# imironhead/ml_super_resolution

Hardware: AMD Instinct MI355X
Metric: VDSR-20 training patches/sec (41x41, batch 256 per GPU); fwd HR megapixels/sec alongside (higher is better)
Workload: dtype f32; 1 GPU; BASELINE configs[2]: VDSR 20-layer 3x3x64 residual, RGB, batch 256x41x41 per GPU, fwd+bwd+TF-Adam, random-init weights; global_batch=256, patch=41, parallelism=dp1

## Files before the change

ml_super_resolution_amd/csrc/conv_inst_c4.hip:

```cpp
#include "launchers.h"
namespace srx {
bool launch_conv_c4(const ConvKey& k, const ConvArgs& a, int grid, size_t lds, hipStream_t s, hipError_t* err) {
    SRX_CONV_CASE(3, 3, 4, 4, false, 2)
    SRX_CONV_CASE(3, 3, 4, 4, true, 2)
    SRX_CONV_CASE(3, 3, 4, 2, false, 2)
    SRX_CONV_CASE(3, 3, 4, 2, true, 2)
    SRX_CONV_CASE(3, 3, 4, 1, false, 2)
    SRX_CONV_CASE(5, 5, 4, 4, false, 2)
    SRX_CONV_CASE(5, 5, 4, 4, true, 2)
    SRX_CONV_CASE(5, 5, 4, 2, false, 2)
    SRX_CONV_CASE(5, 5, 4, 2, true, 2)
    SRX_CONV_CASE(9, 9, 4, 4, false, 2)
    SRX_CONV_CASE(9, 9, 4, 4, true, 2)
    return false;
}
}
```

ml_super_resolution_amd/csrc/conv_narrow.hip:

```cpp
#include "launchers.h"
namespace srx {
typedef float f32x3 __attribute__((ext_vector_type(3)));
typedef unsigned u32x3v __attribute__((ext_vector_type(3)));

template <int CTRL>
__device__ __forceinline__ float dpp_add(float v) {
    const int moved = __builtin_amdgcn_update_dpp(0, __float_as_int(v), CTRL, 0xf, 0xf, false);
    return v + __int_as_float(moved);
}

struct PixWalk {
    int n, oh, ow;
    __device__ __forceinline__ void init(unsigned p, int OH, int OW) {
        const unsigned t = p / (unsigned)OW;
        ow = (int)(p - t * (unsigned)OW);
        n = (int)(t / (unsigned)OH);
        oh = (int)(t - (unsigned)n * (unsigned)OH);
    }
    __device__ __forceinline__ void step16(int OH, int OW) { step(16, OH, OW); }
    __device__ __forceinline__ void step(int d, int OH, int OW) {
        ow += d;
        while (ow >= OW) {
            ow -= OW;
            oh += 1;
            if (oh == OH) { oh = 0; n += 1; }
        }
    }
};
template <int KH, int KW>
__device__ __forceinline__ void tap_offsets(int (&off)[KH * KW], const PixWalk& q, bool live, int H, int W, int pad_t, int pad_l,
                                            int PB, int lane_b) {
    const int centre = ((q.n * H + q.oh - pad_t) * W + (q.ow - pad_l)) * PB + lane_b;
    bool rok[KH], cok[KW];
#pragma unroll
    for (int kh = 0; kh < KH; ++kh) rok[kh] = live && (unsigned)(q.oh + kh - pad_t) < (unsigned)H;
#pragma unroll
    for (int kw = 0; kw < KW; ++kw) cok[kw] = (unsigned)(q.ow + kw - pad_l) < (unsigned)W;
#pragma unroll
    for (int kh = 0; kh < KH; ++kh)
#pragma unroll
        for (int kw = 0; kw < KW; ++kw)
            off[kh * KW + kw] = (rok[kh] && cok[kw]) ? centre + (kh * W + kw) * PB : kOobOffset;
}

template <int KH, int KW, int CIN, int CO>
__global__ __launch_bounds__(256) void conv_narrow_kernel(const ConvArgs a, long total_px, int iters) {
    static_assert(CIN == 64, "16 lanes x 4 channels per pixel");
    constexpr int TAPS = KH * KW;
    const int c4 = threadIdx.x & 15;
    const int sub = threadIdx.x >> 4;
    float wr[TAPS][4][CO];
#pragma unroll
    for (int t = 0; t < TAPS; ++t)
#pragma unroll
        for (int e = 0; e < 4; ++e)
#pragma unroll
            for (int c = 0; c < CO; ++c) wr[t][e][c] = a.w[((size_t)t * CIN + 4 * c4 + e) * CO + c];
    float bias[CO];
#pragma unroll
    for (int c = 0; c < CO; ++c) bias[c] = a.bias ? a.bias[c] : 0.0f;
    const __amdgpu_buffer_rsrc_t xrs = __builtin_amdgcn_make_buffer_rsrc(const_cast<float*>(a.x), 0,
                                                                         a.N * a.H * a.W * CIN * 4, 0x00020000);
    const unsigned p0 = blockIdx.x * (unsigned)iters * 16u + sub;
    PixWalk q;
    q.init(p0 < (unsigned)total_px ? p0 : 0u, a.OH, a.OW);
    for (int it = 0; it < iters; ++it, q.step16(a.OH, a.OW)) {
        const unsigned p = p0 + (unsigned)it * 16u;
        const bool live = p < (unsigned)total_px;
        int off[TAPS];
        tap_offsets<KH, KW>(off, q, live, a.H, a.W, a.pad_t, a.pad_l, CIN * 4, 16 * c4);
        f32x4 v[TAPS];
#pragma unroll
        for (int tp = 0; tp < TAPS; ++tp)
            v[tp] = __builtin_bit_cast(f32x4, __builtin_amdgcn_raw_buffer_load_b128(xrs, off[tp], 0, 0));
        float acc[CO];
#pragma unroll
        for (int c = 0; c < CO; ++c) acc[c] = 0.0f;
#pragma unroll
        for (int tp = 0; tp < TAPS; ++tp)
#pragma unroll
            for (int e = 0; e < 4; ++e)
#pragma unroll
                for (int c = 0; c < CO; ++c) acc[c] = fmaf(v[tp][e], wr[tp][e][c], acc[c]);
#pragma unroll
        for (int c = 0; c < CO; ++c) {
            float r = acc[c];
            r = dpp_add<0xB1>(r);
            r = dpp_add<0x4E>(r);
            r = dpp_add<0x124>(r);
            r = dpp_add<0x128>(r);
            acc[c] = r;
        }
        if (live && c4 < CO) {
            float r = (c4 == 0) ? acc[0] : (c4 == 1 ? acc[1 < CO ? 1 : 0] : acc[2 < CO ? 2 : 0]);
            r = act_apply(r + ((c4 == 0) ? bias[0] : (c4 == 1 ? bias[1 < CO ? 1 : 0] : bias[2 < CO ? 2 : 0])), a.act);
            const size_t o = (size_t)p * CO + c4;
            if (a.skip) r += a.skip[o];
            if (a.post_relu) r = act_apply(r, a.post_relu);
            a.y[o] = r;
        }
    }
}

template <int KH, int KW, bool NOUT, int CW = 64>
__global__ __launch_bounds__(256) void wgrad_narrow_kernel(const WgradArgs a, long total_px, int iters) {
    constexpr int TAPS = KH * KW, CN = 3;
    constexpr int LPP = CW / 4;
    constexpr int PPI = 256 / LPP;
    constexpr int NB = NOUT ? CN : 4;
    constexpr int NV = TAPS * 4 * CN + NB;
    __shared__ float red[4 * NV * LPP];
    const int c4 = threadIdx.x & (LPP - 1);
    const int sub = threadIdx.x / LPP;
    const int wave = threadIdx.x >> 6;
    float acc[NV];
#pragma unroll
    for (int i = 0; i < NV; ++i) acc[i] = 0.0f;
    const __amdgpu_buffer_rsrc_t xrs = __builtin_amdgcn_make_buffer_rsrc(
        const_cast<float*>(a.x), 0, a.N * a.H * a.W * (NOUT ? CW : CN) * 4, 0x00020000);
    const __amdgpu_buffer_rsrc_t drs = __builtin_amdgcn_make_buffer_rsrc(
        const_cast<float*>(a.dpre), 0, a.N * a.OH * a.OW * (NOUT ? CN : CW) * 4, 0x00020000);
    const unsigned p0 = blockIdx.x * (unsigned)iters * (unsigned)PPI + sub;
    PixWalk q;
    q.init(p0 < (unsigned)total_px ? p0 : 0u, a.OH, a.OW);
    for (int it = 0; it < iters; ++it, q.step(PPI, a.OH, a.OW)) {
        const unsigned p = p0 + (unsigned)it * (unsigned)PPI;
        const bool live = p < (unsigned)total_px;
        int off[TAPS];
        tap_offsets<KH, KW>(off, q, live, a.H, a.W, a.pad_t, a.pad_l, (NOUT ? CW : CN) * 4, NOUT ? 16 * c4 : 0);
        if constexpr (NOUT) {
            const f32x3 d = __builtin_bit_cast(f32x3, __builtin_amdgcn_raw_buffer_load_b96(drs, live ? (int)(p * CN * 4) : kOobOffset, 0, 0));
            f32x4 v[TAPS];
#pragma unroll
            for (int tp = 0; tp < TAPS; ++tp)
                v[tp] = __builtin_bit_cast(f32x4, __builtin_amdgcn_raw_buffer_load_b128(xrs, off[tp], 0, 0));
#pragma unroll
            for (int tp = 0; tp < TAPS; ++tp)
#pragma unroll
                for (int e = 0; e < 4; ++e)
#pragma unroll
                    for (int c = 0; c < CN; ++c) acc[(tp * 4 + e) * CN + c] = fmaf(v[tp][e], d[c], acc[(tp * 4 + e) * CN + c]);
#pragma unroll
            for (int c = 0; c < CN; ++c) acc[TAPS * 4 * CN + c] += d[c];
        } else {
            const f32x4 d = __builtin_bit_cast(f32x4, __builtin_amdgcn_raw_buffer_load_b128(
                drs, live ? (int)((p * CW + 4 * c4) * 4) : kOobOffset, 0, 0));
            f32x3 v[TAPS];
#pragma unroll
            for (int tp = 0; tp < TAPS; ++tp)
                v[tp] = __builtin_bit_cast(f32x3, __builtin_amdgcn_raw_buffer_load_b96(xrs, off[tp], 0, 0));
#pragma unroll
            for (int tp = 0; tp < TAPS; ++tp)
#pragma unroll
                for (int cn = 0; cn < CN; ++cn)
#pragma unroll
                    for (int e = 0; e < 4; ++e) acc[(tp * CN + cn) * 4 + e] = fmaf(v[tp][cn], d[e], acc[(tp * CN + cn) * 4 + e]);
#pragma unroll
            for (int e = 0; e < 4; ++e) acc[TAPS * 4 * CN + e] += d[e];
        }
    }
#pragma unroll
    for (int i = 0; i < NV; ++i) {
        float r = acc[i];
#pragma unroll
        for (int o = LPP; o < 64; o <<= 1) r += __shfl_xor(r, o);
        if (sub % (64 / LPP) == 0) red[(wave * NV + i) * LPP + c4] = r;
    }
    __syncthreads();
    float* part = a.part + (size_t)blockIdx.x * a.part_stride;
    const int wn = TAPS * CW * CN;
    for (int q = threadIdx.x; q < NV * LPP; q += 256) {
        const int i = q / LPP, l = q % LPP;
        const float r = (red[(0 * NV + i) * LPP + l] + red[(1 * NV + i) * LPP + l]) +
                        (red[(2 * NV + i) * LPP + l] + red[(3 * NV + i) * LPP + l]);
        if (i < TAPS * 4 * CN) {
            int idx;
            if constexpr (NOUT) {
                const int c = i % CN, te = i / CN, e = te & 3, tp = te >> 2;
                idx = (tp * CW + 4 * l + e) * CN + c;
            } else {
                const int e = i & 3, tc = i >> 2;
                idx = tc * CW + 4 * l + e;
            }
            part[idx] = r;
        } else {
            const int b = i - TAPS * 4 * CN;
            if constexpr (NOUT) {
                if (l == 0) part[wn + b] = r;
            } else {
                part[wn + 4 * l + b] = r;
            }
        }
    }
}

bool launch_wgrad_narrow(const ConvKey& k, const WgradArgs& a, int grid, hipStream_t s, hipError_t* err) {
    if (k.kh != 3 || k.kw != 3) return false;
    const bool nout = a.Cin == 64 && a.Cout == 3, nin = a.Cin == 3 && a.Cout == 64, nin32 = a.Cin == 3 && a.Cout == 32;
    if (!nout && !nin && !nin32) return false;
    const long total = (long)a.N * a.OH * a.OW;
    if (total >= (1L << 31) - 4096 || (long)a.N * a.H * a.W * 64 * 4 >= (1L << 31) - 4096 || total * 64 * 4 >= (1L << 31) - 4096)
        return false;
    const long ppi = nin32 ? 32 : 16;
    const int iters = (int)((total + ppi * grid - 1) / (ppi * grid));
    if (nout)
        hipLaunchKernelGGL((wgrad_narrow_kernel<3, 3, true>), dim3(grid), dim3(256), 0, s, a, total, iters);
    else if (nin)
        hipLaunchKernelGGL((wgrad_narrow_kernel<3, 3, false>), dim3(grid), dim3(256), 0, s, a, total, iters);
    else
        hipLaunchKernelGGL((wgrad_narrow_kernel<3, 3, false, 32>), dim3(grid), dim3(256), 0, s, a, total, iters);
    *err = hipGetLastError();
    return true;
}

bool launch_conv_narrow(const ConvKey& k, const ConvArgs& a, hipStream_t s, hipError_t* err) {
    if (k.wt || a.Cout != 3 || a.mask) return false;
    if ((long)a.N * a.H * a.W * a.Cin * 4 >= (1L << 31) - 4096) return false;
    const long total = (long)a.N * a.OH * a.OW;
    int iters = 16;
    while (iters > 1 && total / (16L * iters) < 2048) iters >>= 1;
    const long blocks = (total + 16L * iters - 1) / (16L * iters);
    if (total >= (1L << 31) - 4096) return false;
    if (k.kh == 3 && k.kw == 3 && a.Cin == 64) {
        hipLaunchKernelGGL((conv_narrow_kernel<3, 3, 64, 3>), dim3((unsigned)blocks), dim3(256), 0, s, a, total, iters);
    } else {
        return false;
    }
    *err = hipGetLastError();
    return true;
}
}
```

Baseline: 20090 patches/s.

## Add streaming 3-channel input conv kernel and one-load DPP weight-gradient path

Adds a dedicated streaming kernel for the first 3x3 conv (3 input channels to 64 outputs). Weights are held in registers, and each of the 16 lanes in a row loads a single tap, which is broadcast across the row with DPP row_newbcast fused multiply-adds. Loads are software-pipelined four chunks deep and the grid is sized to twice the CU count. The narrow weight-gradient kernel gets a similar path: one tap load per lane, row broadcast, and packed FMAs, replacing the nine-tap loads. This cuts redundant global loads for the thin-channel layer in exchange for inline assembly and hardware-specific DPP modes.

```diff
diff --git a/ml_super_resolution_amd/csrc/conv_c4_stream.h b/ml_super_resolution_amd/csrc/conv_c4_stream.h
--- /dev/null
+++ b/ml_super_resolution_amd/csrc/conv_c4_stream.h
@@ -0,0 +1,195 @@
+#pragma once
+#include <stdlib.h>
+#include "launchers.h"
+
+namespace srx {
+
+typedef float f32x3s __attribute__((ext_vector_type(3)));
+typedef unsigned u32x4s __attribute__((ext_vector_type(4)));
+
+template <bool WT>
+__global__ __launch_bounds__(256, 2) void conv_c4_stream_kernel(const ConvArgs a, int total_px, int cpb, int rem) {
+    constexpr int TAPS = 9, CN = 3, CW = 64;
+    const int c4 = threadIdx.x & 15;
+    const int sub = threadIdx.x >> 4;
+    float wr[TAPS][CN][4];
+    if constexpr (!WT) {
+#pragma unroll
+        for (int t = 0; t < TAPS; ++t)
+#pragma unroll
+            for (int ci = 0; ci < CN; ++ci) {
+                const f32x4 v = *reinterpret_cast<const f32x4*>(a.w + (t * CN + ci) * CW + 4 * c4);
+#pragma unroll
+                for (int e = 0; e < 4; ++e) wr[t][ci][e] = v[e];
+            }
+    } else {
+#pragma unroll
+        for (int t = 0; t < TAPS; ++t) {
+            const float* wp = a.w + ((TAPS - 1 - t) * CW + 4 * c4) * CN;
+            const f32x4 v0 = *reinterpret_cast<const f32x4*>(wp), v1 = *reinterpret_cast<const f32x4*>(wp + 4),
+                        v2 = *reinterpret_cast<const f32x4*>(wp + 8);
+            const float f[12] = {v0[0], v0[1], v0[2], v0[3], v1[0], v1[1], v1[2], v1[3], v2[0], v2[1], v2[2], v2[3]};
+#pragma unroll
+            for (int ci = 0; ci < CN; ++ci)
+#pragma unroll
+                for (int e = 0; e < 4; ++e) wr[t][ci][e] = f[e * CN + ci];
+        }
+    }
+    f32x4 bias4 = {0.f, 0.f, 0.f, 0.f};
+    if (a.bias)
+#pragma unroll
+        for (int e = 0; e < 4; ++e) bias4[e] = a.bias[4 * c4 + e];
+
+    const int wide_bytes = total_px * CW * 4;
+    const __amdgpu_buffer_rsrc_t xrs = __builtin_amdgcn_make_buffer_rsrc(const_cast<float*>(a.x), 0, a.N * a.H * a.W * CN * 4, 0x00020000);
+    const __amdgpu_buffer_rsrc_t yrs = __builtin_amdgcn_make_buffer_rsrc(a.y, 0, wide_bytes, 0x00020000);
+    const float* auxp = a.mask ? a.mask : a.skip;
+    const __amdgpu_buffer_rsrc_t ars = __builtin_amdgcn_make_buffer_rsrc(const_cast<float*>(auxp), 0, auxp ? wide_bytes : 0, 0x00020000);
+
+    const int b = blockIdx.x;
+    const int first = b * cpb + (b < rem ? b : rem), count = cpb + (b < rem ? 1 : 0);
+    const int kh = (c4 < TAPS) ? c4 / 3 : 0, kw = (c4 < TAPS) ? c4 - 3 * (c4 / 3) : 0;
+    const bool has_aux = auxp != nullptr;
+
+    int p = first * 16 + sub;
+    int ow, oh, n;
+    {
+        const unsigned pp = (p < total_px) ? (unsigned)p : 0u;
+        const unsigned t = pp / (unsigned)a.OW;
+        ow = (int)(pp - t * (unsigned)a.OW);
+        n = (int)(t / (unsigned)a.OH);
+        oh = (int)(t - (unsigned)n * (unsigned)a.OH);
+    }
+    const auto step16 = [&] {
+        ow += 16;
+        if (a.OW >= 16) {
+            const bool r = ow >= a.OW;
+            ow -= r ? a.OW : 0;
+            oh += r ? 1 : 0;
+            const bool i = oh == a.OH;
+            oh = i ? 0 : oh;
+            n += i ? 1 : 0;
+        } else {
+            while (ow >= a.OW) {
+                ow -= a.OW;
+                oh += 1;
+                if (oh == a.OH) { oh = 0; n += 1; }
+            }
+        }
+    };
+    const auto load_tap = [&](bool live) {
+        const int ih = oh + kh - a.pad_t, iw = ow + kw - a.pad_l;
+        const bool ok = live && c4 < TAPS && (unsigned)ih < (unsigned)a.H && (unsigned)iw < (unsigned)a.W;
+        return __builtin_bit_cast(f32x3s, __builtin_amdgcn_raw_buffer_load_b96(xrs, ok ? ((n * a.H + ih) * a.W + iw) * 12 : kOobOffset, 0, 0));
+    };
+    const auto finish = [&](const f32x3s tap, const f32x4 aux, int wo) {
+        float v0 = bias4[0], v1 = bias4[1], v2 = bias4[2], v3 = bias4[3];
+#define SRX_STREAM_TAP(T)                                                                                              \
+        asm volatile("s_nop 1\n\t"                                                                                     \
+                     "v_fmac_f32_dpp %0, %4, %7 row_newbcast:" #T " row_mask:0xf bank_mask:0xf\n\t"                     \
+                     "v_fmac_f32_dpp %1, %4, %8 row_newbcast:" #T " row_mask:0xf bank_mask:0xf\n\t"                     \
+                     "v_fmac_f32_dpp %2, %4, %9 row_newbcast:" #T " row_mask:0xf bank_mask:0xf\n\t"                     \
+                     "v_fmac_f32_dpp %3, %4, %10 row_newbcast:" #T " row_mask:0xf bank_mask:0xf\n\t"                    \
+                     "v_fmac_f32_dpp %0, %5, %11 row_newbcast:" #T " row_mask:0xf bank_mask:0xf\n\t"                    \
+                     "v_fmac_f32_dpp %1, %5, %12 row_newbcast:" #T " row_mask:0xf bank_mask:0xf\n\t"                    \
+                     "v_fmac_f32_dpp %2, %5, %13 row_newbcast:" #T " row_mask:0xf bank_mask:0xf\n\t"                    \
+                     "v_fmac_f32_dpp %3, %5, %14 row_newbcast:" #T " row_mask:0xf bank_mask:0xf\n\t"                    \
+                     "v_fmac_f32_dpp %0, %6, %15 row_newbcast:" #T " row_mask:0xf bank_mask:0xf\n\t"                    \
+                     "v_fmac_f32_dpp %1, %6, %16 row_newbcast:" #T " row_mask:0xf bank_mask:0xf\n\t"                    \
+                     "v_fmac_f32_dpp %2, %6, %17 row_newbcast:" #T " row_mask:0xf bank_mask:0xf\n\t"                    \
+                     "v_fmac_f32_dpp %3, %6, %18 row_newbcast:" #T " row_mask:0xf bank_mask:0xf"                         \
+                     : "+v"(v0), "+v"(v1), "+v"(v2), "+v"(v3)                                                          \
+                     : "v"(tap[0]), "v"(tap[1]), "v"(tap[2]),                                                          \
+                       "v"(wr[T][0][0]), "v"(wr[T][0][1]), "v"(wr[T][0][2]), "v"(wr[T][0][3]),                         \
+                       "v"(wr[T][1][0]), "v"(wr[T][1][1]), "v"(wr[T][1][2]), "v"(wr[T][1][3]),                         \
+                       "v"(wr[T][2][0]), "v"(wr[T][2][1]), "v"(wr[T][2][2]), "v"(wr[T][2][3]));
+        SRX_STREAM_TAP(0) SRX_STREAM_TAP(1) SRX_STREAM_TAP(2) SRX_STREAM_TAP(3) SRX_STREAM_TAP(4)
+        SRX_STREAM_TAP(5) SRX_STREAM_TAP(6) SRX_STREAM_TAP(7) SRX_STREAM_TAP(8)
+#undef SRX_STREAM_TAP
+        f32x4 v = {v0, v1, v2, v3};
+        if (a.act == ACT_RELU) v = act_apply4(v, ACT_RELU, 0.0f);
+        if (a.mask) {
+            if (a.mask_act == ACT_RELU) v = act_grad4(v, aux, ACT_RELU, 0.0f);
+        } else {
+            v += aux;
+        }
+        __builtin_amdgcn_raw_buffer_store_b128(__builtin_bit_cast(u32x4s, v), yrs, wo, 0, 0);
+    };
+
+    constexpr int U = 4;
+    const int whole = total_px / 16 - first;
+    const int ng = (count < whole ? count : (whole > 0 ? whole : 0)) / U;
+    const f32x4 zero4 = {0.f, 0.f, 0.f, 0.f};
+    f32x3s tap[U];
+    f32x4 aux[U];
+    int wo = (p * CW + 4 * c4) * 4;
+    if (ng > 0) {
+#pragma unroll
+        for (int u = 0; u < U; ++u) {
+            tap[u] = load_tap(true);
+            aux[u] = has_aux ? __builtin_bit_cast(f32x4, __builtin_amdgcn_raw_buffer_load_b128(ars, wo, u * 4096, 0)) : zero4;
+            step16();
+        }
+    }
+    __builtin_amdgcn_s_waitcnt(0);
+    for (int g = 0; g < ng; ++g) {
+        f32x3s tap_n[U];
+        f32x4 aux_n[U];
+        if (g + 1 < ng) {
+#pragma unroll
+            for (int u = 0; u < U; ++u) {
+                tap_n[u] = load_tap(true);
+                aux_n[u] = has_aux ? __builtin_bit_cast(f32x4, __builtin_amdgcn_raw_buffer_load_b128(ars, wo + U * 4096, u * 4096, 0)) : zero4;
+                step16();
+            }
+        } else {
+#pragma unroll
+            for (int u = 0; u < U; ++u) { tap_n[u] = f32x3s{0.f, 0.f, 0.f}; aux_n[u] = zero4; }
+        }
+#pragma unroll
+        for (int u = 0; u < U; ++u) finish(tap[u], aux[u], wo + u * 4096);
+#pragma unroll
+        for (int u = 0; u < U; ++u) { tap[u] = tap_n[u]; aux[u] = aux_n[u]; }
+        wo += U * 4096;
+        p += U * 16;
+    }
+    for (int c = ng * U; c < count; ++c) {
+        const bool live = p < total_px;
+        const int wl = live ? wo : kOobOffset;
+        const f32x3s t1 = load_tap(live);
+        const f32x4 a1 = has_aux ? __builtin_bit_cast(f32x4, __builtin_amdgcn_raw_buffer_load_b128(ars, wl, 0, 0)) : zero4;
+        finish(t1, a1, wl);
+        step16();
+        wo += 4096;
+        p += 16;
+    }
+}
+
+inline bool launch_conv_c4_stream(const ConvKey& k, const ConvArgs& a, hipStream_t s, hipError_t* err) {
+    static const bool on = [] { const char* e = getenv("SRX_C4_STREAM"); return !e || atoi(e) != 0; }();
+    if (!on || k.kh != 3 || k.kw != 3 || k.cinp != 4 || k.nch != 4 || a.Cin != 3 || a.Cout != 64 || a.stride != 1 || a.d2s_r) return false;
+    if ((a.act != ACT_NONE && a.act != ACT_RELU) || a.post_relu || (a.mask && a.skip) ||
+        (a.mask && a.mask_act != ACT_NONE && a.mask_act != ACT_RELU)) return false;
+    const long total = (long)a.N * a.OH * a.OW;
+    if (total * 64 * 4 >= (1L << 31) - (1L << 24) || (long)a.N * a.H * a.W * 3 * 4 >= (1L << 31) - 4096) return false;
+    int dev = 0, cus = 0;
+    if ((*err = hipGetDevice(&dev)) != hipSuccess) return true;
+    static thread_local int cu_of[64] = {0};
+    if (dev >= 0 && dev < 64 && cu_of[dev]) {
+        cus = cu_of[dev];
+    } else {
+        if ((*err = hipDeviceGetAttribute(&cus, hipDeviceAttributeMultiprocessorCount, dev)) != hipSuccess) return true;
+        if (dev >= 0 && dev < 64) cu_of[dev] = cus;
+    }
+    const long chunks = (total + 15) / 16;
+    const int grid = (int)(chunks < 2L * cus ? chunks : 2L * cus);
+    const int cpb = (int)(chunks / grid), rem = (int)(chunks % grid);
+    if (k.wt)
+        hipLaunchKernelGGL(conv_c4_stream_kernel<true>, dim3(grid), dim3(256), 0, s, a, (int)total, cpb, rem);
+    else
+        hipLaunchKernelGGL(conv_c4_stream_kernel<false>, dim3(grid), dim3(256), 0, s, a, (int)total, cpb, rem);
+    *err = hipGetLastError();
+    return true;
+}
+
+}
diff --git a/ml_super_resolution_amd/csrc/conv_inst_c4.hip b/ml_super_resolution_amd/csrc/conv_inst_c4.hip
--- a/ml_super_resolution_amd/csrc/conv_inst_c4.hip
+++ b/ml_super_resolution_amd/csrc/conv_inst_c4.hip
@@ -1,6 +1,8 @@
 #include "launchers.h"
+#include "conv_c4_stream.h"
 namespace srx {
 bool launch_conv_c4(const ConvKey& k, const ConvArgs& a, int grid, size_t lds, hipStream_t s, hipError_t* err) {
+    if (launch_conv_c4_stream(k, a, s, err)) return true;
     SRX_CONV_CASE(3, 3, 4, 4, false, 2)
     SRX_CONV_CASE(3, 3, 4, 4, true, 2)
     SRX_CONV_CASE(3, 3, 4, 2, false, 2)
diff --git a/ml_super_resolution_amd/csrc/conv_narrow.hip b/ml_super_resolution_amd/csrc/conv_narrow.hip
--- a/ml_super_resolution_amd/csrc/conv_narrow.hip
+++ b/ml_super_resolution_amd/csrc/conv_narrow.hip
@@ -7,6 +7,11 @@
 __device__ __forceinline__ float dpp_add(float v) {
     const int moved = __builtin_amdgcn_update_dpp(0, __float_as_int(v), CTRL, 0xf, 0xf, false);
     return v + __int_as_float(moved);
+}
+
+template <int T>
+__device__ __forceinline__ float row_bcast(float v) {
+    return __int_as_float(__builtin_amdgcn_update_dpp(0, __float_as_int(v), 0x150 + T, 0xf, 0xf, false));
 }
 
 struct PixWalk {
@@ -123,7 +128,44 @@
     const unsigned p0 = blockIdx.x * (unsigned)iters * (unsigned)PPI + sub;
     PixWalk q;
     q.init(p0 < (unsigned)total_px ? p0 : 0u, a.OH, a.OW);
-    for (int it = 0; it < iters; ++it, q.step(PPI, a.OH, a.OW)) {
+    constexpr bool ONE_LOAD = !NOUT && LPP == 16 && TAPS == 9;
+    if constexpr (ONE_LOAD) {
+        const int kh = (c4 * 11) >> 5, kw = c4 - 3 * kh;
+        const auto load = [&](unsigned p, bool live, f32x4& d, f32x3& t) {
+            const int ih = q.oh + kh - a.pad_t, iw = q.ow + kw - a.pad_l;
+            const bool ok = live && c4 < TAPS && (unsigned)ih < (unsigned)a.H && (unsigned)iw < (unsigned)a.W;
+            t = __builtin_bit_cast(f32x3, __builtin_amdgcn_raw_buffer_load_b96(xrs, ok ? ((q.n * a.H + ih) * a.W + iw) * CN * 4 : kOobOffset, 0, 0));
+            d = __builtin_bit_cast(f32x4, __builtin_amdgcn_raw_buffer_load_b128(drs, live ? (int)((p * CW + 4 * c4) * 4) : kOobOffset, 0, 0));
+        };
+        f32x4 d;
+        f32x3 t;
+        load(p0, iters > 0 && p0 < (unsigned)total_px, d, t);
+        for (int it = 0; it < iters; ++it) {
+            q.step(PPI, a.OH, a.OW);
+            const unsigned pn = p0 + (unsigned)(it + 1) * (unsigned)PPI;
+            f32x4 dn;
+            f32x3 tn;
+            load(pn, it + 1 < iters && pn < (unsigned)total_px, dn, tn);
+            const f32x2 d01 = {d[0], d[1]}, d23 = {d[2], d[3]};
+#define SRX_WGRAD_TAP(T)                                                                                       \
+            _Pragma("unroll") for (int cn = 0; cn < CN; ++cn) {                                                \
+                const float xv = row_bcast<T>(t[cn]);                                                          \
+                const f32x2 x2 = {xv, xv};                                                                     \
+                float* r = acc + (T * CN + cn) * 4;                                                            \
+                const f32x2 r01 = __builtin_elementwise_fma(x2, d01, f32x2{r[0], r[1]});                       \
+                const f32x2 r23 = __builtin_elementwise_fma(x2, d23, f32x2{r[2], r[3]});                       \
+                r[0] = r01[0]; r[1] = r01[1]; r[2] = r23[0]; r[3] = r23[1];                                    \
+            }
+            SRX_WGRAD_TAP(0) SRX_WGRAD_TAP(1) SRX_WGRAD_TAP(2) SRX_WGRAD_TAP(3) SRX_WGRAD_TAP(4)
+            SRX_WGRAD_TAP(5) SRX_WGRAD_TAP(6) SRX_WGRAD_TAP(7) SRX_WGRAD_TAP(8)
+#undef SRX_WGRAD_TAP
+#pragma unroll
+            for (int e = 0; e < 4; ++e) acc[TAPS * 4 * CN + e] += d[e];
+            d = dn;
+            t = tn;
+        }
+    }
+    for (int it = 0; !ONE_LOAD && it < iters; ++it, q.step(PPI, a.OH, a.OW)) {
         const unsigned p = p0 + (unsigned)it * (unsigned)PPI;
         const bool live = p < (unsigned)total_px;
         int off[TAPS];
```

Measured after the change: 20180 patches/s, median of 6. Within noise of the previous version (+0.5%).

## Double-buffer loads in narrow conv and wgrad kernels, size grid to one resident round

Applied to the files above, without the earlier changes.

The narrow 64->3 conv kernel now issues the next iteration's tap and skip loads before computing the current one, using two register buffers. It also specialises the epilogue by activation type and loads the skip tensor through a buffer resource. The 64->3 wgrad kernel gets the same double buffering, with accumulators packed as float2 and pinned by empty asm so the compiler keeps the schedule. The pixel walker's row wrap becomes branch-free, and the conv grid is sized from queried occupancy so all workgroups fit in one resident wave. The aim is to hide memory latency in these narrow layers, at the cost of extra registers that could reduce occupancy.

```diff
diff --git a/ml_super_resolution_amd/csrc/conv_narrow.hip b/ml_super_resolution_amd/csrc/conv_narrow.hip
--- a/ml_super_resolution_amd/csrc/conv_narrow.hip
+++ b/ml_super_resolution_amd/csrc/conv_narrow.hip
@@ -1,4 +1,6 @@
 #include "launchers.h"
+#include <atomic>
+#include <type_traits>
 namespace srx {
 typedef float f32x3 __attribute__((ext_vector_type(3)));
 typedef unsigned u32x3v __attribute__((ext_vector_type(3)));
@@ -7,6 +9,20 @@
 __device__ __forceinline__ float dpp_add(float v) {
     const int moved = __builtin_amdgcn_update_dpp(0, __float_as_int(v), CTRL, 0xf, 0xf, false);
     return v + __int_as_float(moved);
+}
+
+typedef float f32x2 __attribute__((ext_vector_type(2)));
+template <int I, int N>
+__device__ __forceinline__ void pin_here(f32x2 (&a)[N]) {
+    if constexpr (I + 16 <= N) {
+        asm volatile("" : "+v"(a[I]), "+v"(a[I + 1]), "+v"(a[I + 2]), "+v"(a[I + 3]), "+v"(a[I + 4]), "+v"(a[I + 5]), "+v"(a[I + 6]),
+                          "+v"(a[I + 7]), "+v"(a[I + 8]), "+v"(a[I + 9]), "+v"(a[I + 10]), "+v"(a[I + 11]), "+v"(a[I + 12]),
+                          "+v"(a[I + 13]), "+v"(a[I + 14]), "+v"(a[I + 15]) : : "memory");
+        pin_here<I + 16, N>(a);
+    } else if constexpr (I < N) {
+        asm volatile("" : "+v"(a[I]) : : "memory");
+        pin_here<I + 1, N>(a);
+    }
 }
 
 struct PixWalk {
@@ -17,14 +33,19 @@
         n = (int)(t / (unsigned)OH);
         oh = (int)(t - (unsigned)n * (unsigned)OH);
     }
-    __device__ __forceinline__ void step16(int OH, int OW) { step(16, OH, OW); }
-    __device__ __forceinline__ void step(int d, int OH, int OW) {
+    __device__ __forceinline__ void step(int d, int OH, int OW, bool many) {
         ow += d;
-        while (ow >= OW) {
-            ow -= OW;
-            oh += 1;
-            if (oh == OH) { oh = 0; n += 1; }
-        }
+        wrap(OH, OW);
+        if (many)
+            while (ow >= OW) wrap(OH, OW);
+    }
+    __device__ __forceinline__ void wrap(int OH, int OW) {
+        const bool row = ow >= OW;
+        ow -= row ? OW : 0;
+        oh += row ? 1 : 0;
+        const bool img = oh == OH;
+        oh = img ? 0 : oh;
+        n += img ? 1 : 0;
     }
 };
 template <int KH, int KW>
@@ -43,7 +64,7 @@
             off[kh * KW + kw] = (rok[kh] && cok[kw]) ? centre + (kh * W + kw) * PB : kOobOffset;
 }
 
-template <int KH, int KW, int CIN, int CO>
+template <int KH, int KW, int CIN, int CO, int EPI>
 __global__ __launch_bounds__(256) void conv_narrow_kernel(const ConvArgs a, long total_px, int iters) {
     static_assert(CIN == 64, "16 lanes x 4 channels per pixel");
     constexpr int TAPS = KH * KW;
@@ -59,20 +80,30 @@
     float bias[CO];
 #pragma unroll
     for (int c = 0; c < CO; ++c) bias[c] = a.bias ? a.bias[c] : 0.0f;
+    const float my_bias = (c4 == 0) ? bias[0] : (c4 == 1 ? bias[1 < CO ? 1 : 0] : bias[2 < CO ? 2 : 0]);
     const __amdgpu_buffer_rsrc_t xrs = __builtin_amdgcn_make_buffer_rsrc(const_cast<float*>(a.x), 0,
                                                                          a.N * a.H * a.W * CIN * 4, 0x00020000);
+    const bool has_skip = a.skip != nullptr;
+    const __amdgpu_buffer_rsrc_t srs = __builtin_amdgcn_make_buffer_rsrc(const_cast<float*>(a.skip), 0,
+                                                                         has_skip ? (int)total_px * CO * 4 : 0, 0x00020000);
     const unsigned p0 = blockIdx.x * (unsigned)iters * 16u + sub;
+    const bool many = a.OW < 16;
     PixWalk q;
     q.init(p0 < (unsigned)total_px ? p0 : 0u, a.OH, a.OW);
-    for (int it = 0; it < iters; ++it, q.step16(a.OH, a.OW)) {
+    const auto issue = [&](f32x4 (&v)[TAPS], float& sk, int it) {
+        const unsigned p = p0 + (unsigned)it * 16u;
+        const bool live = it < iters && p < (unsigned)total_px;
+        int off[TAPS];
+        tap_offsets<KH, KW>(off, q, live, a.H, a.W, a.pad_t, a.pad_l, CIN * 4, 16 * c4);
+#pragma unroll
+        for (int tp = 0; tp < TAPS; ++tp)
+            v[tp] = __builtin_bit_cast(f32x4, __builtin_amdgcn_raw_buffer_load_b128(xrs, off[tp], 0, 0));
+        sk = __builtin_bit_cast(float, __builtin_amdgcn_raw_buffer_load_b32(srs, (live && c4 < CO) ? (int)((p * CO + c4) * 4) : kOobOffset, 0, 0));
+        q.step(16, a.OH, a.OW, many);
+    };
+    const auto finish = [&](const f32x4 (&v)[TAPS], float sk, int it) {
         const unsigned p = p0 + (unsigned)it * 16u;
         const bool live = p < (unsigned)total_px;
-        int off[TAPS];
-        tap_offsets<KH, KW>(off, q, live, a.H, a.W, a.pad_t, a.pad_l, CIN * 4, 16 * c4);
-        f32x4 v[TAPS];
-#pragma unroll
-        for (int tp = 0; tp < TAPS; ++tp)
-            v[tp] = __builtin_bit_cast(f32x4, __builtin_amdgcn_raw_buffer_load_b128(xrs, off[tp], 0, 0));
         float acc[CO];
 #pragma unroll
         for (int c = 0; c < CO; ++c) acc[c] = 0.0f;
@@ -91,14 +122,29 @@
             r = dpp_add<0x128>(r);
             acc[c] = r;
         }
-        if (live && c4 < CO) {
-            float r = (c4 == 0) ? acc[0] : (c4 == 1 ? acc[1 < CO ? 1 : 0] : acc[2 < CO ? 2 : 0]);
-            r = act_apply(r + ((c4 == 0) ? bias[0] : (c4 == 1 ? bias[1 < CO ? 1 : 0] : bias[2 < CO ? 2 : 0])), a.act);
-            const size_t o = (size_t)p * CO + c4;
-            if (a.skip) r += a.skip[o];
-            if (a.post_relu) r = act_apply(r, a.post_relu);
-            a.y[o] = r;
-        }
+        float r = (c4 == 0) ? acc[0] : (c4 == 1 ? acc[1 < CO ? 1 : 0] : acc[2 < CO ? 2 : 0]);
+        r += my_bias;
+        if (EPI == 1) r = fmaxf(r, 0.0f);
+        if (EPI == 2) r = act_apply(r, a.act);
+        if (has_skip) r += sk;
+        if (EPI == 2 && a.post_relu) r = act_apply(r, a.post_relu);
+        asm volatile("" : "+v"(r));
+        if (live && c4 < CO) a.y[(size_t)p * CO + c4] = r;
+    };
+    f32x4 va[TAPS], vb[TAPS];
+    float ska, skb;
+    int it = 0;
+    issue(va, ska, 0);
+    if (iters & 1) {
+        finish(va, ska, 0);
+        issue(va, ska, 1);
+        it = 1;
+    }
+    for (; it < iters; it += 2) {
+        issue(vb, skb, it + 1);
+        finish(va, ska, it);
+        issue(va, ska, it + 2);
+        finish(vb, skb, it + 1);
     }
 }
 
@@ -113,55 +159,89 @@
     const int c4 = threadIdx.x & (LPP - 1);
     const int sub = threadIdx.x / LPP;
     const int wave = threadIdx.x >> 6;
-    float acc[NV];
-#pragma unroll
-    for (int i = 0; i < NV; ++i) acc[i] = 0.0f;
+    f32x2 acc2[(NV + 1) / 2];
+#define acc(i) acc2[(i) >> 1][(i) & 1]
+#pragma unroll
+    for (int i = 0; i < (NV + 1) / 2; ++i) acc2[i] = f32x2{0.0f, 0.0f};
     const __amdgpu_buffer_rsrc_t xrs = __builtin_amdgcn_make_buffer_rsrc(
         const_cast<float*>(a.x), 0, a.N * a.H * a.W * (NOUT ? CW : CN) * 4, 0x00020000);
     const __amdgpu_buffer_rsrc_t drs = __builtin_amdgcn_make_buffer_rsrc(
         const_cast<float*>(a.dpre), 0, a.N * a.OH * a.OW * (NOUT ? CN : CW) * 4, 0x00020000);
     const unsigned p0 = blockIdx.x * (unsigned)iters * (unsigned)PPI + sub;
+    const bool many = a.OW < PPI;
     PixWalk q;
     q.init(p0 < (unsigned)total_px ? p0 : 0u, a.OH, a.OW);
-    for (int it = 0; it < iters; ++it, q.step(PPI, a.OH, a.OW)) {
+    using XV = typename std::conditional<NOUT, f32x4, f32x3>::type;
+    using DV = typename std::conditional<NOUT, f32x3, f32x4>::type;
+    const auto issue = [&](XV (&v)[TAPS], DV& d, int it) {
         const unsigned p = p0 + (unsigned)it * (unsigned)PPI;
-        const bool live = p < (unsigned)total_px;
+        const bool live = it < iters && p < (unsigned)total_px;
         int off[TAPS];
         tap_offsets<KH, KW>(off, q, live, a.H, a.W, a.pad_t, a.pad_l, (NOUT ? CW : CN) * 4, NOUT ? 16 * c4 : 0);
         if constexpr (NOUT) {
-            const f32x3 d = __builtin_bit_cast(f32x3, __builtin_amdgcn_raw_buffer_load_b96(drs, live ? (int)(p * CN * 4) : kOobOffset, 0, 0));
-            f32x4 v[TAPS];
+            d = __builtin_bit_cast(f32x3, __builtin_amdgcn_raw_buffer_load_b96(drs, live ? (int)(p * CN * 4) : kOobOffset, 0, 0));
 #pragma unroll
             for (int tp = 0; tp < TAPS; ++tp)
                 v[tp] = __builtin_bit_cast(f32x4, __builtin_amdgcn_raw_buffer_load_b128(xrs, off[tp], 0, 0));
-#pragma unroll
-            for (int tp = 0; tp < TAPS; ++tp)
-#pragma unroll
-                for (int e = 0; e < 4; ++e)
-#pragma unroll
-                    for (int c = 0; c < CN; ++c) acc[(tp * 4 + e) * CN + c] = fmaf(v[tp][e], d[c], acc[(tp * 4 + e) * CN + c]);
-#pragma unroll
-            for (int c = 0; c < CN; ++c) acc[TAPS * 4 * CN + c] += d[c];
         } else {
-            const f32x4 d = __builtin_bit_cast(f32x4, __builtin_amdgcn_raw_buffer_load_b128(
+            d = __builtin_bit_cast(f32x4, __builtin_amdgcn_raw_buffer_load_b128(
                 drs, live ? (int)((p * CW + 4 * c4) * 4) : kOobOffset, 0, 0));
-            f32x3 v[TAPS];
 #pragma unroll
             for (int tp = 0; tp < TAPS; ++tp)
                 v[tp] = __builtin_bit_cast(f32x3, __builtin_amdgcn_raw_buffer_load_b96(xrs, off[tp], 0, 0));
+        }
+        q.step(PPI, a.OH, a.OW, many);
+    };
+    const auto add = [&](const XV (&v)[TAPS], const DV& d) {
+        if constexpr (NOUT) {
 #pragma unroll
             for (int tp = 0; tp < TAPS; ++tp)
 #pragma unroll
+                for (int e = 0; e < 4; ++e)
+#pragma unroll
+                    for (int c = 0; c < CN; ++c) acc((tp * 4 + e) * CN + c) = fmaf(v[tp][e], d[c], acc((tp * 4 + e) * CN + c));
+#pragma unroll
+            for (int c = 0; c < CN; ++c) acc(TAPS * 4 * CN + c) += d[c];
+        } else {
+#pragma unroll
+            for (int tp = 0; tp < TAPS; ++tp)
+#pragma unroll
                 for (int cn = 0; cn < CN; ++cn)
 #pragma unroll
-                    for (int e = 0; e < 4; ++e) acc[(tp * CN + cn) * 4 + e] = fmaf(v[tp][cn], d[e], acc[(tp * CN + cn) * 4 + e]);
-#pragma unroll
-            for (int e = 0; e < 4; ++e) acc[TAPS * 4 * CN + e] += d[e];
+                    for (int e = 0; e < 4; ++e) acc((tp * CN + cn) * 4 + e) = fmaf(v[tp][cn], d[e], acc((tp * CN + cn) * 4 + e));
+#pragma unroll
+            for (int e = 0; e < 4; ++e) acc(TAPS * 4 * CN + e) += d[e];
+        }
+    };
+    if constexpr (NOUT) {
+        XV va[TAPS], vb[TAPS];
+        DV da, db;
+        int it = 0;
+        issue(va, da, 0);
+        if (iters & 1) {
+            add(va, da);
+            issue(va, da, 1);
+            it = 1;
+        }
+        for (; it < iters; it += 2) {
+            issue(vb, db, it + 1);
+            add(va, da);
+            pin_here<0>(acc2);
+            issue(va, da, it + 2);
+            add(vb, db);
+            pin_here<0>(acc2);
+        }
+    } else {
+        XV v[TAPS];
+        DV d;
+        for (int it = 0; it < iters; ++it) {
+            issue(v, d, it);
+            add(v, d);
         }
     }
 #pragma unroll
     for (int i = 0; i < NV; ++i) {
-        float r = acc[i];
+        float r = acc(i);
 #pragma unroll
         for (int o = LPP; o < 64; o <<= 1) r += __shfl_xor(r, o);
         if (sub % (64 / LPP) == 0) red[(wave * NV + i) * LPP + c4] = r;
@@ -194,6 +274,8 @@
     }
 }
 
+#undef acc
+
 bool launch_wgrad_narrow(const ConvKey& k, const WgradArgs& a, int grid, hipStream_t s, hipError_t* err) {
     if (k.kh != 3 || k.kw != 3) return false;
     const bool nout = a.Cin == 64 && a.Cout == 3, nin = a.Cin == 3 && a.Cout == 64, nin32 = a.Cin == 3 && a.Cout == 32;
@@ -213,20 +295,47 @@
     return true;
 }
 
+template <auto Kernel>
+hipError_t resident_workgroups(int* n) {
+    static std::atomic<int> cached[64];
+    int dev = 0, cus = 0, per_cu = 0;
+    hipError_t e = hipGetDevice(&dev);
+    if (e != hipSuccess) return e;
+    const bool keep = dev >= 0 && dev < 64;
+    if (keep && (*n = cached[dev].load(std::memory_order_relaxed)) > 0) return hipSuccess;
+    if ((e = hipDeviceGetAttribute(&cus, hipDeviceAttributeMultiprocessorCount, dev)) != hipSuccess) return e;
+    if ((e = hipOccupancyMaxActiveBlocksPerMultiprocessor(&per_cu, Kernel, 256, 0)) != hipSuccess) return e;
+    if (cus <= 0 || per_cu <= 0) return hipErrorInvalidValue;
+    *n = cus * per_cu;
+    if (keep) cached[dev].store(*n, std::memory_order_relaxed);
+    return hipSuccess;
+}
+
+template <auto Kernel>
+hipError_t launch_one_round(const ConvArgs& a, long total, hipStream_t s) {
+    int resident = 0;
+    const hipError_t e = resident_workgroups<Kernel>(&resident);
+    if (e != hipSuccess) return e;
+    const long groups = (total + 15) / 16;
+    if (groups <= 0) return hipErrorInvalidValue;
+    const int iters = (int)((groups + resident - 1) / resident);
+    const long grid = (groups + iters - 1) / iters;
+    hipLaunchKernelGGL(Kernel, dim3((unsigned)grid), dim3(256), 0, s, a, total, iters);
+    return hipGetLastError();
+}
+
 bool launch_conv_narrow(const ConvKey& k, const ConvArgs& a, hipStream_t s, hipError_t* err) {
     if (k.wt || a.Cout != 3 || a.mask) return false;
     if ((long)a.N * a.H * a.W * a.Cin * 4 >= (1L << 31) - 4096) return false;
     const long total = (long)a.N * a.OH * a.OW;
-    int iters = 16;
-    while (iters > 1 && total / (16L * iters) < 2048) iters >>= 1;
-    const long blocks = (total + 16L * iters - 1) / (16L * iters);
     if (total >= (1L << 31) - 4096) return false;
-    if (k.kh == 3 && k.kw == 3 && a.Cin == 64) {
-        hipLaunchKernelGGL((conv_narrow_kernel<3, 3, 64, 3>), dim3((unsigned)blocks), dim3(256), 0, s, a, total, iters);
-    } else {
-        return false;
-    }
-    *err = hipGetLastError();
+    if (k.kh != 3 || k.kw != 3 || a.Cin != 64) return false;
+    if (a.act == ACT_NONE && !a.post_relu)
+        *err = launch_one_round<conv_narrow_kernel<3, 3, 64, 3, 0>>(a, total, s);
+    else if (a.act == ACT_RELU && !a.post_relu)
+        *err = launch_one_round<conv_narrow_kernel<3, 3, 64, 3, 1>>(a, total, s);
+    else
+        *err = launch_one_round<conv_narrow_kernel<3, 3, 64, 3, 2>>(a, total, s);
     return true;
 }
 }
```

After: 20150 patches/s before, 20230 patches/s after (median of 6 runs). About the same (+0.4%).
